# VainF/Diff-Pruning

Hardware: AMD Instinct MI355X
Metric: importance-scored images/sec (UNet fwd+bwd+|w*dL/dw|) (higher is better)
Workload: dtype f32

## Files before the change

diff-pruning_amd/_lib.py:

```python
import ctypes as C
import os

_HERE = os.path.dirname(os.path.abspath(__file__))
LIB_PATH = os.environ.get('DP_HIP_LIB') or os.path.join(_HERE, 'libdp_hip.so')

c_float_p = C.c_void_p
LL = C.c_longlong


class ConvGeom(C.Structure):
    _fields_ = [(n, C.c_int) for n in ('Ho', 'Wo', 'Hs', 'Ws', 'Hv', 'Wv', 'kw', 'stride', 'sden', 'pad_t', 'pad_l',
                                       'ups', 'c_split', '_pad')] + [('x1_img_stride', LL), ('x2_img_stride', LL)]


class ConvGemmParams(C.Structure):
    _fields_ = [('A', C.c_void_p), ('a_bs', LL), ('lda', C.c_int), ('a_kc', C.c_int),
                ('X1', C.c_void_p), ('X2', C.c_void_p), ('x_bs', LL),
                ('a_bytes', C.c_uint), ('x1_bytes', C.c_uint), ('x2_bytes', C.c_uint), ('_pad0', C.c_uint),
                ('g', ConvGeom),
                ('M', C.c_int), ('C', C.c_int), ('NPIX', C.c_int), ('ntaps', C.c_int), ('batches', C.c_int),
                ('tile', C.c_int),
                ('out', C.c_void_p), ('o_img_stride', LL), ('o_bs', LL),
                ('alpha', C.c_float), ('post_scale', C.c_float),
                ('bias', C.c_void_p), ('tadd', C.c_void_p), ('tadd_stride', LL),
                ('res', C.c_void_p), ('r_img_stride', LL),
                ('accumulate', C.c_int), ('ksplit', C.c_int), ('ws', C.c_void_p), ('x_guard', C.c_int), ('act', C.c_int),
                ('tile_counters', C.c_void_p)]


class NtGemmParams(C.Structure):
    _fields_ = [('A', C.c_void_p), ('a_bs', LL), ('a_img_stride', LL),
                ('X1', C.c_void_p), ('X2', C.c_void_p), ('x_bs', LL),
                ('a_bytes', C.c_uint), ('x1_bytes', C.c_uint), ('x2_bytes', C.c_uint), ('_pad0', C.c_uint),
                ('g', ConvGeom),
                ('M', C.c_int), ('C', C.c_int), ('NCOLS', C.c_int), ('ntaps', C.c_int), ('P', C.c_int),
                ('batches', C.c_int), ('splits', C.c_int), ('p_per_split', C.c_int), ('tile', C.c_int),
                ('batched', C.c_int),
                ('out', C.c_void_p), ('o_bs', LL), ('ldo', C.c_int), ('accumulate', C.c_int),
                ('alpha', C.c_float), ('merge', C.c_int), ('ocs', LL),
                ('o_tap_stride', LL), ('o_col_stride', C.c_int), ('xcd', C.c_int), ('col_bias', C.c_void_p)]


class AttentionParams(C.Structure):
    _fields_ = [('q', C.c_void_p), ('k', C.c_void_p), ('v', C.c_void_p), ('o', C.c_void_p),
                ('q_bs', LL), ('k_bs', LL), ('v_bs', LL), ('o_bs', LL),
                ('N', C.c_int), ('heads', C.c_int), ('d', C.c_int), ('dv', C.c_int), ('T', C.c_int), ('scale', C.c_float),
                ('variant', C.c_int), ('_pad', C.c_int)]


class Dropout(C.Structure):
    _fields_ = [('thr24', C.c_uint), ('scale', C.c_float), ('seed', C.c_ulonglong), ('site', C.c_uint), ('step', C.c_uint),
                ('n_off', LL), ('step_dev', C.c_void_p)]


class ScoreMember(C.Structure):
    _fields_ = [('w', C.c_void_p), ('g', C.c_void_p), ('R', C.c_int), ('C', C.c_int), ('T', C.c_int), ('dim', C.c_int),
                ('mode', C.c_int), ('blk0', C.c_int), ('full_off', LL), ('col_off', LL), ('idx_off', LL)]


class SliceItem(C.Structure):
    _fields_ = [('src', C.c_void_p), ('dst', C.c_void_p), ('R', C.c_int), ('C', C.c_int), ('T', C.c_int), ('dim', C.c_int),
                ('n_keep', C.c_int), ('blk0', C.c_int), ('nblk', C.c_int), ('_pad', C.c_int), ('keep_off', LL)]


class PackItem(C.Structure):
    _fields_ = [('W', C.c_void_p), ('dst', C.c_void_p), ('Co', C.c_int), ('Ci', C.c_int), ('taps', C.c_int), ('mode', C.c_int),
                ('ld', C.c_int), ('blk0', C.c_int), ('nblk', C.c_int), ('_pad', C.c_int)]


class Ups9Params(C.Structure):
    _fields_ = [('U', C.c_void_p), ('dy', C.c_void_p), ('dx', C.c_void_p), ('dy_img_stride', LL), ('dx_img_stride', LL),
                ('u_bytes', C.c_uint), ('dy_bytes', C.c_uint)] + [(n, C.c_int) for n in ('ldu', 'N', 'M', 'K', 'H', 'W',
                                                                                         'accumulate', 'tile')]


class ColsumItem(C.Structure):
    _fields_ = [('src', C.c_void_p), ('dst', C.c_void_p), ('N', C.c_int), ('C', C.c_int), ('wstride', C.c_int),
                ('woff', C.c_int), ('accumulate', C.c_int), ('ld', C.c_int)]


_vp, _i, _f, _ll = C.c_void_p, C.c_int, C.c_float, LL
_dr = C.POINTER(Dropout)

SIGNATURES = {
    'dp_conv_gemm': [C.POINTER(ConvGemmParams), _vp],
    'dp_conv_wino': [C.POINTER(ConvGemmParams), _vp],
    'dp_conv_wino_supported': [C.POINTER(ConvGemmParams)],
    'dp_conv_splitk_epilogue': [C.POINTER(ConvGemmParams), _vp],
    'dp_pack_weight_wino': [_vp, _i, _i, _i, _vp, _i, _vp],
    'dp_conv_wino2d': [C.POINTER(ConvGemmParams), _vp],
    'dp_conv_wino2d_supported': [C.POINTER(ConvGemmParams)],
    'dp_pack_weight_wino2d': [_vp, _i, _i, _i, _vp, _i, _vp],
    'dp_conv_wino43': [C.POINTER(ConvGemmParams), _vp],
    'dp_conv_wino43_supported': [C.POINTER(ConvGemmParams)],
    'dp_pack_weight_wino43': [_vp, _i, _i, _vp, _i, _vp],
    'dp_wgrad_wino': [C.POINTER(NtGemmParams), _vp],
    'dp_wgrad_wino2d': [C.POINTER(NtGemmParams), _vp],
    'dp_wgrad_wino2d_supported': [C.POINTER(NtGemmParams)],
    'dp_wgrad_wino_supported': [C.POINTER(NtGemmParams)],
    'dp_nt_gemm': [C.POINTER(NtGemmParams), _vp],
    'dp_splitk_reduce': [_vp, _ll, _i, _vp, _ll, _i, _vp],
    'dp_splitk_reduce_taps': [_vp, _ll, _i, _vp, _ll, _i, _i, _vp],
    'dp_pack_weight': [_vp, _i, _i, _i, _i, _vp, _i, _vp],
    'dp_pack_weight_batch': [C.POINTER(PackItem), _i, _vp],
    'dp_groupnorm_silu_fwd': [_vp, _vp, _i, _ll, _ll, _vp, _vp, _i, _i, _i, _i, _f, _i, _vp, _ll, _vp, _dr, _vp],
    'dp_groupnorm_silu_bwd': [_vp, _vp, _i, _ll, _ll, _vp, _vp, _vp, _vp, _ll, _i, _i, _i, _i, _i, _vp, _ll, _vp, _ll,
                              _vp, _ll, _vp, _dr, _vp, _vp],
    'dp_groupnorm_silu_fwd_split': [_vp, _vp, _i, _ll, _ll, _vp, _vp, _i, _i, _i, _i, _f, _i, _vp, _ll, _vp, _i, _vp, _dr,
                                    _vp],
    'dp_groupnorm_silu_bwd_split': [_vp, _vp, _i, _ll, _ll, _vp, _vp, _vp, _vp, _ll, _i, _i, _i, _i, _i, _vp, _ll, _vp, _ll,
                                    _vp, _ll, _vp, _i, _vp, _dr, _vp],
    'dp_colsum_accum': [_vp, _i, _i, _i, _i, _vp, _i, _vp],
    'dp_colsum_accum_batch': [C.POINTER(ColsumItem), _i, _vp],
    'dp_rowsum_nc': [_vp, _ll, _i, _i, _i, _vp, _vp],
    'dp_silu_fwd': [_vp, _vp, _ll, _vp],
    'dp_silu_bwd': [_vp, _vp, _vp, _ll, _i, _vp],
    'dp_axpby': [_vp, _f, _vp, _f, _ll, _vp],
    'dp_copy_strided': [_vp, _ll, _vp, _ll, _i, _ll, _i, _vp],
    'dp_attention_fwd': [C.POINTER(AttentionParams), _vp],
    'dp_attention_fwd_supported': [_i, _i, _i],
    'dp_softmax_fwd': [_vp, _vp, _ll, _i, _vp],
    'dp_softmax_bwd': [_vp, _vp, _vp, _ll, _i, _f, _vp],
    'dp_timestep_embedding': [_vp, _i, _i, _i, _f, _f, _vp, _vp],
    'dp_add_noise': [_vp, _vp, _vp, _vp, _i, _ll, _vp, _vp],
    'dp_mse_fwd_bwd': [_vp, _vp, _ll, _f, _vp, _vp, _i, _vp, _vp],
    'dp_kd_fwd_bwd': [_vp, _vp, _vp, _ll, _f, _f, _f, _vp, _vp, _i, _vp],
    'dp_kd_terms': [_vp, _i, _f, _f, _f, _vp, _vp],
    'dp_early_exit_update': [_vp, _f, _vp, _vp, _i, _vp],
    'dp_zero_if_stopped': [_vp, _ll, _vp, _vp],
    'dp_early_exit_update_ratio': [_vp, _f, _vp, _vp, _i, _vp],
    'dp_randn_philox': [_vp, _ll, _ll, C.c_ulonglong, C.c_uint, C.c_uint, _vp],
    'dp_sum_partials': [_vp, _i, _f, _vp, _vp],
    'dp_downsum2x2': [_vp, _ll, _i, _i, _i, _i, _vp, _ll, _vp],
    'dp_upsample2x': [_vp, _ll, _i, _i, _i, _i, _vp, _ll, _vp],
    'dp_interleave2x2': [_vp, _ll, _ll, _i, _i, _i, _i, _vp, _ll, _vp, _ll, _vp],
    'dp_deinterleave2x2': [_vp, _ll, _i, _i, _i, _i, _vp, _ll, _ll, _vp],
    'dp_ups_weff': [_vp, _ll, _vp, _vp],
    'dp_ups_wfold': [_vp, _ll, _vp, _i, _vp],
    'dp_ups9_u': [_vp, _ll, _vp, _vp],
    'dp_ups9_dgrad': [C.POINTER(Ups9Params), _vp],
    'dp_ups9_dgrad_supported': [C.POINTER(Ups9Params)],
    'dp_wg_reduce': [_vp, _vp, _i, _i, _i, _i, _i, _vp, _i, _vp, _vp],
    'dp_gather_add': [_vp, _vp, _i, _vp, _vp],
    'dp_group_score': [C.POINTER(ScoreMember), _i, _i, _vp, _vp, _vp, _vp],
    'dp_slice_batch': [C.POINTER(SliceItem), _i, _vp, _vp],
    'dp_sumsq_partials': [_vp, _ll, _vp, _i, _vp],
    'dp_clip_coef': [_vp, _i, _f, _vp, _vp, _vp],
    'dp_adam_ema': [_vp, _vp, _vp, _vp, _vp, _ll, _vp, _f, _f, _f, _f, _f, _f, _f, _vp],
    'dp_set_step_scalars': [_vp, _f, _f, _f, C.c_uint, _vp],
    'dp_adamw_ema': [_vp, _vp, _vp, _vp, _vp, _ll, _vp, _f, _f, _f, _f, _f, _f, _f, _f, _vp],
    'dp_embedding_bwd': [_vp, _vp, _i, _i, _vp, _vp],
    'dp_ema_update': [_vp, _vp, _ll, _f, _vp],
    'dp_adam_ema_dev': [_vp, _vp, _vp, _vp, _vp, _ll, _vp, _vp, _f, _f, _f, _f, _vp],
    'dp_ddim_step': [_vp, _vp, _vp, _f, _f, _f, _i, _f, _vp, _ll, _vp],
    'dp_ddpm_step': [_vp, _vp, _vp, _f, _f, _f, _f, _f, _i, _f, _vp, _ll, _vp],
    'dp_denoise_step': [_vp, _vp, _vp, _i, _f, _f, _f, _f, _f, _f, _vp, _vp, _ll, _vp],
    'dp_image_to_u8': [_vp, _ll, _i, _i, _i, _i, _i, _vp, _vp],
    'dp_cfg_denoise_step': [_vp, _vp, _vp, _f, _i, _vp, _vp, _vp, _f, _f, _f, _f, _f, _f, _vp, _vp, _vp, _vp, _ll, _vp],
    'dp_dropout_apply': [_vp, _ll, _vp, _ll, _i, _ll, _dr, _vp],
    'dp_dropout_mask': [_vp, _ll, _ll, _dr, _vp],
    'dp_layernorm_fwd': [_vp, _ll, _vp, _vp, _i, _i, _i, _f, _vp, _ll, _vp, _vp],
    'dp_layernorm_bwd': [_vp, _ll, _vp, _vp, _vp, _ll, _i, _i, _i, _vp, _ll, _vp, _ll, _vp, _vp],
    'dp_geglu_fwd': [_vp, _i, _ll, _vp, _vp],
    'dp_geglu_bwd': [_vp, _vp, _i, _ll, _vp, _vp],
    'dp_add_rowvec': [_vp, _ll, _vp, _i, _i, _i, _vp, _ll, _vp],
    'dp_q_sample': [_vp, _vp, _vp, _vp, _vp, _i, _ll, _vp, _vp],
    'dp_cfg_combine': [_vp, _vp, _f, _vp, _ll, _vp],
    'dp_u8_to_float': [_vp, _i, _i, _i, _i, _i, _vp, _ll, _i, C.c_uint, _i, _dr, _vp],
    'dp_pool2d': [_vp, _ll, _i, _i, _i, _i, _i, _i, _i, _i, _vp, _ll, _vp],
    'dp_resize_bilinear': [_vp, _ll, _i, _i, _i, _i, _i, _i, _f, _f, _vp, _vp],
    'dp_ssim': [_vp, _vp, _i, _i, _i, _i, _f, _vp, _vp, _vp],
    'dp_ssim_workspace': [_i, _i, _i, _i],
    'dp_mse_per_image': [_vp, _vp, _i, _ll, _vp, _vp],
    'dp_vq_blocks': [_ll],
    'dp_vq_quantize': [_vp, _ll, _i, _i, _ll, _vp, _i, _vp, _ll, _vp, _vp, _vp],
    'dp_vq_loss': [_vp, _i, C.c_double, _vp, _vp],
    'dp_replay_build': [_vp, C.POINTER(C.c_void_p)],
    'dp_replay_launch': [_vp, _vp, _vp],
    'dp_replay_info': [_vp, C.POINTER(C.c_int)],
    'dp_replay_free': [_vp],
    'dp_version': [],
    'dp_launch_count': [],
    'dp_recent_launches': [C.POINTER(C.c_char_p), _i],
}

_lib = None


class DpHipError(RuntimeError):
    code = None


def load():
    global _lib
# ... 20 lines not shown
```

diff-pruning_amd/csrc/ups9.hip:

```cpp
#include "dp_common.h"

#define U9_RSRC_FLAGS 0x00020000
#define U9_OOB 0x80000000u

__device__ __forceinline__ __amdgpu_buffer_rsrc_t u9_rsrc(const float* base, unsigned bytes) {
    return __builtin_amdgcn_make_buffer_rsrc((void*)base, 0, (int)bytes, U9_RSRC_FLAGS);
}
__device__ __forceinline__ float u9_bload(__amdgpu_buffer_rsrc_t r, unsigned byte_off) {
    asm volatile("" : "+v"(byte_off));
    return __builtin_bit_cast(float, __builtin_amdgcn_raw_buffer_load_b32(r, (int)byte_off, 0, 0));
}
__device__ __forceinline__ f32x4 u9_bload4(__amdgpu_buffer_rsrc_t r, unsigned byte_off) {
    asm volatile("" : "+v"(byte_off));
    return __builtin_bit_cast(f32x4, __builtin_amdgcn_raw_buffer_load_b128(r, (int)byte_off, 0, 0));
}

template <int BM, int BN, int KC, int WM, int WN, int OCC>
__global__ __launch_bounds__(256, OCC) void ups9_dgrad_kernel(const dp_ups9_params p) {
    constexpr int TM = BM / (32 * WM), TN = BN / (32 * WN);
    constexpr int KT = 9 * KC;
    constexpr int PT = BN * KC / 256;
    constexpr int KSTEP = 256 / BN;
    constexpr int MCH = BM / 4;
    constexpr int ACH = KT * MCH;
    constexpr int NA = (ACH + 255) / 256;
    static_assert(WM * WN == 4 && TM >= 1 && TN >= 1 && PT >= 1 && (BN * KC) % 256 == 0 && KT % 2 == 0 && BN <= 256, "tile");
    __shared__ __attribute__((aligned(16))) float As[KT * BM];
    __shared__ __attribute__((aligned(16))) float Ts[KT * BN];

    const int tid = threadIdx.x;
    const int lane = tid & 63;
    const int wave = __builtin_amdgcn_readfirstlane(tid >> 6);
    const int li = lane & 31, lk = lane >> 5;
    const int wm0 = (wave / WN) * (TM * 32), wn0 = (wave % WN) * (TN * 32);
    const int H = p.H, W = p.W, HW = H * W, W2 = 2 * W, HW4 = 4 * HW;
    const int K = p.K, M = p.M;
    const int NPIX = p.N * HW;
    const int MT = (M + BM - 1) / BM;
    const int PTILES = (NPIX + BN - 1) / BN;
    int mt, ptile;
    {
        const int b = blockIdx.x;
        if (!(PTILES & 7)) {
            const int xcd = b & 7, slot = b >> 3;
            mt = slot % MT;
            ptile = (slot / MT) * 8 + xcd;
        } else {
            mt = b % MT;
            ptile = b / MT;
        }
    }
    const int m0 = mt * BM, px0 = ptile * BN;

// ... 101 lines not shown
    }

#pragma unroll
    for (int tn = 0; tn < TN; ++tn) {
        const int pixel = px0 + wn0 + tn * 32 + li;
        if (pixel >= NPIX) continue;
        const int n = pixel / HW, rem = pixel - n * HW;
        float* o = p.dx + (long long)n * p.dx_img_stride + rem;
#pragma unroll
        for (int tm = 0; tm < TM; ++tm)
#pragma unroll
            for (int r = 0; r < 16; ++r) {
                const int row = m0 + wm0 + tm * 32 + (r & 3) + 8 * (r >> 2) + 4 * lk;
                if (row < M) {
                    float* q = o + (long long)row * HW;
                    *q = p.accumulate ? *q + acc[tm][tn][r] : acc[tm][tn][r];
                }
            }
    }
}

static const int u9_bn[3] = {32, 64, 128};

extern "C" int dp_ups9_dgrad_supported(const dp_ups9_params* pp) {
    const dp_ups9_params& p = *pp;
    if (!p.U || !p.dy || !p.dx || ((uintptr_t)p.U & 15)) return 0;
    if (p.N < 1 || p.M < 1 || p.K < 1 || p.H < 1 || p.W < 1 || p.tile < 0 || p.tile > 2) return 0;
    if (p.ldu < p.M || (p.ldu & 3)) return 0;
    const long long HW = (long long)p.H * p.W;
    const long long npix = HW * p.N;
    if (npix >= (1ll << 29)) return 0;
    if (9ll * p.K * p.ldu * 4 != (long long)p.u_bytes || p.u_bytes >= 0x80000000u) return 0;
    if (p.dy_img_stride < 4 * HW * p.K || p.dx_img_stride < HW * p.M) return 0;
    const long long dy_need = ((p.N - 1) * p.dy_img_stride + 4 * HW * p.K) * 4;
    if ((long long)p.dy_bytes < dy_need || p.dy_bytes >= 0x80000000u) return 0;
    const long long blocks = ((npix + u9_bn[p.tile] - 1) / u9_bn[p.tile]) * ((p.M + 127) / 128);
    if (blocks >= (1ll << 31)) return 0;
    return 1;
}

extern "C" int dp_ups9_dgrad(const dp_ups9_params* pp, void* stream) {
    if (!dp_ups9_dgrad_supported(pp)) return (int)hipErrorInvalidValue;
    const dp_ups9_params& p = *pp;
    const long long npix = (long long)p.N * p.H * p.W;
    const int bn = u9_bn[p.tile];
    const dim3 grid((unsigned)(((npix + bn - 1) / bn) * ((p.M + 127) / 128)));
    hipStream_t st = (hipStream_t)stream;
    if (p.tile == 0)      DP_LAUNCH((ups9_dgrad_kernel<128, 32, 8, 4, 1, 2>), grid, dim3(256), 0, st, p);
    else if (p.tile == 1) DP_LAUNCH((ups9_dgrad_kernel<128, 64, 4, 2, 2, 3>), grid, dim3(256), 0, st, p);
    else                  DP_LAUNCH((ups9_dgrad_kernel<128, 128, 4, 2, 2, 2>), grid, dim3(256), 0, st, p);
    return DP_LAUNCH_CHECK();
}

__global__ __launch_bounds__(256) void ups9_u_kernel(const float* __restrict__ w, long long M, float* __restrict__ u) {
    for (long long m = (long long)blockIdx.x * 256 + threadIdx.x; m < M; m += (long long)gridDim.x * 256) {
        float g[3][3], t[3][3];
#pragma unroll
        for (int i = 0; i < 9; ++i) g[i / 3][i % 3] = w[m * 9 + i];
#pragma unroll
        for (int c = 0; c < 3; ++c) {
            t[0][c] = g[0][c];
            t[1][c] = (g[0][c] + g[1][c]) + g[2][c];
            t[2][c] = g[2][c];
        }
#pragma unroll
        for (int a = 0; a < 3; ++a) {
            u[m * 9 + 3 * a + 0] = t[a][0];
            u[m * 9 + 3 * a + 1] = (t[a][0] + t[a][1]) + t[a][2];
            u[m * 9 + 3 * a + 2] = t[a][2];
        }
    }
}

extern "C" int dp_ups9_u(const float* w, long long M, float* u, void* stream) {
    if (M <= 0) return 0;
    long long nb = (M + 255) / 256;
    if (nb > 4096) nb = 4096;
    DP_LAUNCH(ups9_u_kernel, dim3((unsigned)nb), dim3(256), 0, (hipStream_t)stream, w, M, u);
    return DP_LAUNCH_CHECK();
}
```

diff-pruning_amd/engine.py:

```python
import os

import torch

from . import ops

_SPEC3 = ops.ConvSpec(3, 1, 1, 0)
_SPEC1 = ops.ConvSpec(1, 1, 0, 0)
_SPEC_UP = ops.ConvSpec(3, 1, 1, 1)
UPS_COPY = not os.environ.get('DP_NO_UPS_COPY')
UPS_SUBPIXEL = not os.environ.get('DP_NO_UPS_SUBPIXEL')
_UPS_SPECS = ops.UPS_CLASS_SPECS
S2_PARITY = not os.environ.get('DP_NO_S2_PARITY')
FUSE_QKV_WGRAD = not os.environ.get('DP_NO_FUSED_QKV_WGRAD')
OVERLAP_MIN_WORK = 4_000_000

RES_DIFFUSERS = dict(norm1='.norm1', conv1='.conv1', temb='.time_emb_proj', norm2='.norm2', conv2='.conv2',
                     shortcut='.conv_shortcut', dropout='.dropout')
RES_LDM = dict(norm1='.in_layers.0', conv1='.in_layers.2', temb='.emb_layers.1', norm2='.out_layers.0',
               conv2='.out_layers.3', shortcut='.skip_connection')


SIDE_KEEP_MAX_BYTES = int(float(os.environ.get('DP_SIDE_KEEP_GB', '4')) * (1 << 30))


# ... 362 lines not shown
    def replay_side_stream(self, device):
        if getattr(self, '_replay_side', None) is None or self._replay_side.device != torch.device(device):
            self._replay_side = shared_stream(device, 'replay', self.stream_slot)
        return self._replay_side

    def _join_side(self):
        if self._side is not None:
            torch.cuda.current_stream().wait_stream(self._side)
        self._side_keep.clear()
        self._side_keep_bytes = 0

    def _conv_bwd(self, name, dy, x, x2, spec, in_hw, *, need_dx=True, rows=None, dx_out=None, dx_accumulate=False,
                  alpha=1.0, dx_add=None):
        w = self.P[name + '.weight']

        if rows is None and (name + '.bias') in self.P and self._rows_src is not None and self._rows_src[0].data_ptr() == dy.data_ptr():
            rows = self._rows_of(dy)

        def param_grads(rows):
            ops.conv_wgrad(dy, x, x2, self.G[name + '.weight'], spec, alpha=alpha, accumulate=True)
            if (name + '.bias') in self.P:
                if rows is None:
                    rows = ops.rowsum_nc(dy)
                if alpha != 1.0:
                    rows = rows.contiguous()
                    rows = ops.axpby(rows, alpha, torch.empty_like(rows), 0.0)
                self._colsum(rows, rows.shape[0], rows.shape[1], 1, 0, self.G[name + '.bias'])

        side = self._side_stream(dy, x, x2, rows)
        if side is None:
            param_grads(rows)
        else:
            with torch.cuda.stream(side):
                param_grads(rows)
        if not need_dx:
            return None
        if (S2_PARITY and spec.stride == 2 and spec.k == 3 and not spec.ups and spec.pad in (0, 1) and alpha == 1.0
                and dx_out is None and in_hw[0] == 2 * dy.shape[2] and in_hw[1] == 2 * dy.shape[3]):
            packs = [self.packs.get(name, w, ('s2', ph, pw, spec.pad)) for ph in (0, 1) for pw in (0, 1)]
            return ops.conv_dgrad_s2(dy, packs, w.shape[1], spec, in_hw, add=dx_add)
        wd, ldd = self.packs.get(name, w, 1)
        wino = None
        if w.dim() == 4 and w.shape[2] == 3 and hasattr(ops, 'wino_wanted') and tuple(in_hw) == tuple(dy.shape[2:]):
            wino = self._wino_operand(name, w, 1, w.shape[1], (w.shape[0],), dy.shape[0], dy.shape[2], dy.shape[3], spec)
        dx = ops.conv_dgrad(dy, wd, ldd, w.shape[1], spec, in_hw, alpha=alpha, out=dx_out, accumulate=dx_accumulate,
                            **({'wino': wino} if wino is not None else {}))
        if dx_add is not None:
            ops.copy_strided(dx_add, dx, accumulate=True)
        return dx

    def _ups_conv_fwd(self, name, x):
        w = self.P[name + '.weight']
        N, _, H, W = x.shape
        q = ops.empty_act((4, N, w.shape[0], H, W), x.device)
        for c, spec in enumerate(_UPS_SPECS):
            wp, ld = self.packs.get(name, w, ('up', c, 0))
            ops.conv_forward(x, None, wp, ld, w.shape[0], spec, bias=self.P.get(name + '.bias'), out=q[c])
        return ops.interleave2x2(q)

    def _ups_conv_bwd(self, name, dy, x):
        w = self.P[name + '.weight']
        use9 = hasattr(ops, 'ups9_dgrad_wanted') and ops.ups9_dgrad_wanted(x.shape[0], w.shape[1], w.shape[0], x.shape[2], x.shape[3])
        dyq = None if use9 else ops.deinterleave2x2(dy)
        rows = None
        if (name + '.bias') in self.P and self._rows_src is not None and self._rows_src[0].data_ptr() == dy.data_ptr():
            rows = self._rows_of(dy)

        def param_grads(rows, dyq=dyq):
            if dyq is None:
                dyq = ops.deinterleave2x2(dy)
            gweff = torch.empty((4,) + tuple(w.shape[:2]) + (2, 2), dtype=torch.float32, device=dy.device)
            for c, spec in enumerate(_UPS_SPECS):
                ops.conv_wgrad(dyq[c], x, None, gweff[c], spec, accumulate=False)
            ops.ups_wfold(gweff, self.G[name + '.weight'], accumulate=True)
            if (name + '.bias') in self.P:
                if rows is None:
                    rows = ops.rowsum_nc(dy)
                self._colsum(rows, rows.shape[0], rows.shape[1], 1, 0, self.G[name + '.bias'])

        side = self._side_stream(dy, dyq, x, rows)
        if side is None:
            param_grads(rows)
        else:
            with torch.cuda.stream(side):
                param_grads(rows)
        if use9:
            up, ldu = self.packs.get(name, w, ('up9', 0, 1))
            return ops.ups9_dgrad(dy, up, ldu, w.shape[1])
        dx = None
        for c, spec in enumerate(_UPS_SPECS):
            wd, ldd = self.packs.get(name, w, ('up', c, 1))
            dx = ops.conv_dgrad(dyq[c], wd, ldd, w.shape[1], spec, tuple(x.shape[2:]), out=dx, accumulate=c > 0)
        return dx

    def _gn_param_grads(self, name, pws):
        N, C = pws.shape[0], pws.shape[1]
        self._colsum(pws, N, C, 2, 1, self.G[name + '.weight'])
        self._colsum(pws, N, C, 2, 0, self.G[name + '.bias'])

    def resnet_fwd(self, pre, xa, xb, semb, out_scale, save, names=RES_DIFFUSERS, G=None, eps=None):
        P, cfg = self.P, self.cfg
        G = cfg['norm_num_groups'] if G is None else G
        eps = cfg['norm_eps'] if eps is None else eps
        nm = names
        n1, st1 = ops.groupnorm_fwd(xa, xb, P[pre + nm['norm1'] + '.weight'], P[pre + nm['norm1'] + '.bias'], G, eps, True)
        if self._temb is not None:
# ... 334 lines not shown
```

diff-pruning_amd/ops.py:

```python
import ctypes as C
import os
import math
import torch

from . import _lib as L

_f32 = torch.float32


def _lib():
    return L.load()


_raw_stream = getattr(torch._C, '_cuda_getCurrentRawStream', None)


def _stream():
    if _raw_stream is not None:
        return C.c_void_p(_raw_stream(torch.cuda.current_device()))
    return C.c_void_p(torch.cuda.current_stream().cuda_stream)


def _p(t):
    return None if t is None else C.c_void_p(t.data_ptr())
# ... 619 lines not shown
    npix = HW * N
    if npix >= (1 << 29):
        return False
    if 9 * Cout * ldu * 4 != u_bytes or u_bytes >= _MAX_BYTES:
        return False
    if dy_img_stride < 4 * HW * Cout or dx_img_stride < HW * Cin:
        return False
    if dy_bytes < ((N - 1) * dy_img_stride + 4 * HW * Cout) * 4 or dy_bytes >= _MAX_BYTES:
        return False
    return -(-npix // UPS9_TILE_PIX[tile]) * ((Cin + 127) // 128) < (1 << 31)


def ups9_dgrad_gate(N, Cin, Cout, H, W):
    blocks32 = -(-(N * H * W) // 32) * ((Cin + 127) // 128)
    return blocks32 >= UPS9_GATE_MIN_BLOCKS and max(Cin, Cout) <= UPS9_GATE_MAX_CH


def ups9_dgrad_wanted(N, Cin, Cout, H, W):
    if not UPS9 or min(N, Cin, Cout, H, W) < 1 or N * H * W * 4 * Cout * 4 >= _MAX_BYTES:
        return False
    return ups9_dgrad_gate(N, Cin, Cout, H, W)


def _ups9_params(dy, up, ldu, Cin, out, accumulate, tile):
    sd, so = _chk_act(dy), _chk_act(out)
    N, Cout, H2, W2 = dy.shape
    p = L.Ups9Params()
    p.U, p.dy, p.dx = _p(up), _p(dy), _p(out)
    p.dy_img_stride, p.dx_img_stride = sd, so
    p.u_bytes, p.dy_bytes = up.numel() * 4, _extent_bytes(dy)
    p.ldu, p.N, p.M, p.K, p.H, p.W = ldu, N, Cin, Cout, H2 // 2, W2 // 2
    p.accumulate, p.tile = 1 if accumulate else 0, tile
    return p


def ups9_dgrad(dy, up, ldu, Cin, *, out=None, accumulate=False, tile=None):
    N, Cout, H2, W2 = dy.shape
    assert H2 % 2 == 0 and W2 % 2 == 0
    H, W = H2 // 2, W2 // 2
    if out is None:
        assert not accumulate
        out = empty_act((N, Cin, H, W), dy.device)
    assert out.shape == (N, Cin, H, W)
    if tile is None:
        tile = ups9_tile(N, Cin, H, W)
    p = _ups9_params(dy, up, ldu, Cin, out, accumulate, tile)
    ok = ups9_dgrad_shape_ok(N, Cin, Cout, H, W, p.dy_img_stride, p.dx_img_stride, p.dy_bytes, ldu, p.u_bytes, tile, up.data_ptr())
    assert ok == bool(_lib().dp_ups9_dgrad_supported(C.byref(p))), 'host shape rule and dp_ups9_dgrad_supported disagree'
    if not ok:
        raise ValueError('dp_ups9_dgrad does not take this launch (ups9_dgrad_shape_ok)')
    L.check(_run(lambda: _lib().dp_ups9_dgrad(C.byref(p), _stream()),
                 _UPS9_NAMES[tile],
                 2.0 * Cin * N * H * W * Cout * 9, 4.0 * (dy.numel() + up.numel() + out.numel())), 'dp_ups9_dgrad')
    return out


_ws_cache = {}
WGRAD_BLOCKS = 1024
WGRAD_MIN_PIX = int(os.environ.get('DP_WGRAD_MIN_PIX', '128'))


def _workspace(n, device):
    if torch.cuda.is_current_stream_capturing():
        return torch.empty(max(n, 1), dtype=_f32, device=device)
    key = (device.index if device.index is not None else torch.cuda.current_device(), _stream().value)
    t = _ws_cache.get(key)
    if t is None or t.numel() < n:
        t = torch.empty(max(n, 1 << 22), dtype=_f32, device=device)
        _ws_cache[key] = t
    return t


WGRAD_WINO = os.environ.get('DP_WGRAD_WINO', '1') not in ('0', '')
WGRAD_WINO_MIN_FILL = float(os.environ.get('DP_WGRAD_WINO_MIN_FILL', '0.7'))
WGRAD_WINO_MIN_WORK = int(os.environ.get('DP_WGRAD_WINO_MIN_WORK', '512'))


WGRAD_WINO2D = os.environ.get('DP_WGRAD_WINO2D', '1') not in ('0', '')
WGRAD_WINO2D_BLOCKS = int(os.environ.get('DP_WGRAD_WINO2D_BLOCKS', '512'))
WGRAD_WINO2D_MIN_FILL = float(os.environ.get('DP_WGRAD_WINO2D_MIN_FILL', '0.7'))


def _nt_gemm_params(A, a_img_stride, x, x2, geom, M, Cc, ncols, ntaps, P, splits, pps, tile, alpha, ldo, batch=None):
    p = L.NtGemmParams()
    Z, a_bs, x_bs, batched = batch or (1, 0, 0, 0)
    p.A, p.a_bs, p.a_img_stride = _p(A), a_bs, a_img_stride
    p.X1, p.X2, p.x_bs = _p(x), _p(x2), x_bs
    if batch is None:
        p.a_bytes, p.x1_bytes, p.x2_bytes = _extent_bytes(A), _extent_bytes(x), _extent_bytes(x2)
    else:
        p.a_bytes, p.x1_bytes, p.x2_bytes = M * P * 4, ncols * P * 4, 0
    p.g = geom
    p.M, p.C, p.NCOLS, p.ntaps, p.P = M, Cc, ncols, ntaps, P
    p.batches, p.splits, p.p_per_split, p.tile, p.batched = Z, splits, pps, tile, batched
    p.alpha, p.ldo = alpha, ldo
    return p


def _wgrad_launch(p, gw, accumulate, sym, name, flops, label, taps, device):
    acc = 1 if accumulate else 0
    if p.splits == 1:
        p.out, p.o_bs, p.accumulate = _p(gw), 0, acc
        L.check(_run(lambda: getattr(_lib(), sym)(C.byref(p), _stream()), name, flops), label)
        return gw
    n = gw.numel()
    ws = _workspace(p.splits * n, device)
# ... 894 lines not shown
```

include/dp_hip.h:

```cpp
#ifndef DP_HIP_H
#define DP_HIP_H
#include <stdint.h>
#ifdef __cplusplus
extern "C" {
#endif

typedef struct dp_conv_geom {
    int Ho, Wo, Hs, Ws, Hv, Wv, kw, stride, sden, pad_t, pad_l, ups, c_split, _pad;
    long long x1_img_stride, x2_img_stride;
} dp_conv_geom;

typedef struct dp_conv_gemm_params {
    const float* A; long long a_bs; int lda; int a_kc;
    const float* X1; const float* X2; long long x_bs;
    unsigned a_bytes, x1_bytes, x2_bytes, _pad0;
    dp_conv_geom g;
    int M, C, NPIX, ntaps, batches, tile;
    float* out; long long o_img_stride; long long o_bs;
    float alpha; float post_scale;
    const float* bias; const float* tadd; long long tadd_stride;
    const float* res; long long r_img_stride;
    int accumulate; int ksplit;
    float* ws;
    int x_guard; int act;
// ... 87 lines not shown

int dp_axpby(const float* x, float a, float* y, float b, long long n, void* stream);
int dp_copy_strided(const float* src, long long s_stride, float* dst, long long d_stride, int N, long long per_img, int accumulate, void* stream);

int dp_softmax_fwd(const float* s, float* p, long long rows, int cols, void* stream);
typedef struct dp_attention_params {
    const float* q; const float* k; const float* v; float* o;
    long long q_bs, k_bs, v_bs, o_bs;
    int N, heads, d, dv, T;
    float scale;
    int variant;
    int _pad;
} dp_attention_params;
int dp_attention_fwd(const dp_attention_params* p, void* stream);
int dp_attention_fwd_supported(int T, int d, int dv);
int dp_softmax_bwd(const float* p, const float* dp, float* ds, long long rows, int cols, float scale, void* stream);

int dp_timestep_embedding(const float* t, int B, int dim, int flip_sin_to_cos, float freq_shift, float max_period, float* out, void* stream);

int dp_add_noise(const float* x0, const float* noise, const float* acp, const int64_t* t, int B, long long per_img, float* out, void* stream);

int dp_mse_fwd_bwd(const float* out, const float* noise, long long n, float gscale, float* dout, float* partial, int nblocks,
                   const float* stop_state, void* stream);
int dp_kd_fwd_bwd(const float* out, const float* teacher, const float* noise, long long n, float w_kd, float w_eps, float gscale,
                  float* dout, float* partial, int nblocks, void* stream);
int dp_kd_terms(const float* partial, int nblocks, float w_kd, float w_eps, float scale, float* terms, void* stream);
int dp_early_exit_update(const float* loss, float thr, float* state, float* losses, int max_steps, void* stream);
int dp_zero_if_stopped(float* x, long long n, const float* state, void* stream);
int dp_early_exit_update_ratio(const float* loss, float thr, float* state, float* losses, int max_steps, void* stream);
int dp_sum_partials(const float* partial, int n, float scale, float* dst, void* stream);

int dp_downsum2x2(const float* dy, long long dy_img_stride, int N, int C, int H, int W, float* dx, long long dx_img_stride, void* stream);

int dp_upsample2x(const float* x, long long x_img_stride, int N, int C, int H, int W, float* y, long long y_img_stride, void* stream);

int dp_interleave2x2(const float* q, long long q_class_stride, long long q_img_stride, int N, int C, int Ho, int Wo,
                     const float* add, long long add_img_stride, float* dx, long long dx_img_stride, void* stream);

int dp_deinterleave2x2(const float* y, long long y_img_stride, int N, int C, int Ho, int Wo, float* q,
                       long long q_class_stride, long long q_img_stride, void* stream);

int dp_ups_weff(const float* w, long long M, float* weff, void* stream);
int dp_ups_wfold(const float* gweff, long long M, float* gw, int accumulate, void* stream);

typedef struct dp_ups9_params {
    const float* U; const float* dy; float* dx;
    long long dy_img_stride, dx_img_stride;
    unsigned u_bytes, dy_bytes;
    int ldu, N, M, K, H, W, accumulate, tile;
} dp_ups9_params;
int dp_ups9_u(const float* w, long long M, float* u, void* stream);
int dp_ups9_dgrad(const dp_ups9_params* p, void* stream);
int dp_ups9_dgrad_supported(const dp_ups9_params* p);

int dp_wg_reduce(const float* w, const float* g, int R, int C, int T, int dim, int mode, float* out, int accumulate,
                 float* scratch, void* stream);

int dp_gather_add(const float* src, const int64_t* idx, int n, float* dst, void* stream);

typedef struct dp_score_member {
    const float* w; const float* g;
    int R, C, T, dim, mode, blk0;
    long long full_off, col_off, idx_off;
} dp_score_member;
int dp_group_score(const dp_score_member* members, int n, int n0, const int64_t* idx, float* scratch, float* score, void* stream);
typedef struct dp_slice_item {
    const float* src; float* dst;
    int R, C, T, dim, n_keep, blk0, nblk, _pad;
    long long keep_off;
} dp_slice_item;
int dp_slice_batch(const dp_slice_item* items, int n, const int64_t* keep, void* stream);

int dp_sumsq_partials(const float* x, long long n, float* partial, int nblocks, void* stream);
int dp_set_step_scalars(float* hyper, float lr, float bc1, float bc2, unsigned step, void* stream);
int dp_adam_ema_dev(float* p, const float* g, float* m, float* v, float* ema, long long n, const float* clip_coef,
                    const float* hyper, float b1, float b2, float eps, float ema_decay, void* stream);
int dp_clip_coef(const float* partial, int n, float max_norm, float* norm_out, float* coef_out, void* stream);
int dp_adam_ema(float* p, const float* g, float* m, float* v, float* ema, long long n, const float* clip_coef,
                float lr, float b1, float b2, float eps, float bc1, float bc2, float ema_decay, void* stream);

int dp_adamw_ema(float* p, const float* g, float* m, float* v, float* ema, long long n, const float* clip_coef,
                 float p_scale, float one_minus_b1, float b2, float one_minus_b2, float sqrt_bc2, float eps,
                 float step_size, float ema_decay, void* stream);
int dp_ema_update(float* s, const float* p, long long n, float one_minus_decay, void* stream);
int dp_embedding_bwd(const long long* ids, const float* dctx, int B, int D, float* dW, void* stream);

int dp_ddim_step(const float* x, const float* eps, const float* vnoise, float a_t, float a_prev, float std, int clip,
                 float clip_range, float* out, long long n, void* stream);

int dp_ddpm_step(const float* x, const float* eps, const float* vnoise, float sqrt_a_t, float sqrt_b_t, float c_x0,
                 float c_xt, float sigma, int clip, float clip_range, float* out, long long n, void* stream);

#define DP_DENOISE_MAX_BLOCKS 4096
int dp_denoise_step(const float* x, const float* eps, const float* z, int mode, float p0, float p1, float p2, float p3, float p4,
                    float p5, float* next, float* x0_out, long long n, void* stream);
int dp_image_to_u8(const float* x, long long x_img_stride, int N, int C, int H, int W, int rescaled, unsigned char* out,
                   void* stream);

int dp_cfg_denoise_step(const float* x, const float* e_u, const float* e_c, float scale, int order, const float* h1, const float* h2,
                        const float* h3, float s1m, float sqrt_a_t, float sqrt_a_prev, float c_dir, float sigma, float temperature,
                        const float* z, float* next, float* x0_out, float* eg_out, long long n, void* stream);

int dp_layernorm_fwd(const float* x, long long x_img_stride, const float* gamma, const float* beta, int N, int C, int T,
                     float eps, float* y, long long y_img_stride, float* stats, void* stream);
int dp_layernorm_bwd(const float* x, long long x_img_stride, const float* gamma, const float* stats, const float* dy,
                     long long dy_img_stride, int N, int C, int T, float* dx, long long dx_img_stride, const float* add,
// ... 46 lines not shown
```

Before: 4953.

## Add Winograd-style fused upsample+conv3x3 forward kernel for small-channel layers

Adds a HIP kernel that computes nearest-2x-upsample followed by a 3x3 conv in one pass. It transforms a 3x3 input neighbourhood into 9 Winograd-like terms, multiplies them by pre-transformed weights with MFMA, and writes the 2x2 output pixels directly. This replaces the previous path that ran four per-class GEMMs into an intermediate q buffer and then interleaved them. The new path is gated by block count and channel limits. It adds a pack type ('up9') and extra LDS pressure, and any layer that fails the gate falls back to the old path.

Result: faster. 5017 (median of 6 runs) (+1.3%).

```diff
diff --git a/diff-pruning_amd/_lib.py b/diff-pruning_amd/_lib.py
--- a/diff-pruning_amd/_lib.py
+++ b/diff-pruning_amd/_lib.py
@@ -72,6 +72,11 @@
     _fields_ = [('U', C.c_void_p), ('dy', C.c_void_p), ('dx', C.c_void_p), ('dy_img_stride', LL), ('dx_img_stride', LL),
                 ('u_bytes', C.c_uint), ('dy_bytes', C.c_uint)] + [(n, C.c_int) for n in ('ldu', 'N', 'M', 'K', 'H', 'W',
                                                                                          'accumulate', 'tile')]
+
+
+class Ups9FwdParams(C.Structure):
+    _fields_ = [('U', C.c_void_p), ('x', C.c_void_p), ('bias', C.c_void_p), ('y', C.c_void_p), ('x_img_stride', LL), ('y_img_stride', LL),
+                ('u_bytes', C.c_uint), ('x_bytes', C.c_uint)] + [(n, C.c_int) for n in ('ldu', 'N', 'M', 'K', 'H', 'W')]
 
 
 class ColsumItem(C.Structure):
@@ -140,6 +145,7 @@
     'dp_ups9_u': [_vp, _ll, _vp, _vp],
     'dp_ups9_dgrad': [C.POINTER(Ups9Params), _vp],
     'dp_ups9_dgrad_supported': [C.POINTER(Ups9Params)],
+    'dp_ups9_fwd': [C.POINTER(Ups9FwdParams), _vp],
     'dp_wg_reduce': [_vp, _vp, _i, _i, _i, _i, _i, _vp, _i, _vp, _vp],
     'dp_gather_add': [_vp, _vp, _i, _vp, _vp],
     'dp_group_score': [C.POINTER(ScoreMember), _i, _i, _vp, _vp, _vp, _vp],
diff --git a/diff-pruning_amd/csrc/ups9.hip b/diff-pruning_amd/csrc/ups9.hip
--- a/diff-pruning_amd/csrc/ups9.hip
+++ b/diff-pruning_amd/csrc/ups9.hip
@@ -1,4 +1,6 @@
 #include "dp_common.h"
+
+typedef float f32x2 __attribute__((ext_vector_type(2)));
 
 #define U9_RSRC_FLAGS 0x00020000
 #define U9_OOB 0x80000000u
@@ -206,6 +208,190 @@
     return DP_LAUNCH_CHECK();
 }
 
+template <int BM, int BN, int KC, int OCC>
+__global__ __launch_bounds__(256, OCC) void ups9_fwd_kernel(const dp_ups9_fwd_params p) {
+    constexpr int WN = BN / 32;
+    constexpr int KT = 9 * KC;
+    constexpr int PT = BN * KC / 256;
+    constexpr int KSTEP = 256 / BN;
+    constexpr int MCH = BM / 4;
+    constexpr int ACH = KT * MCH;
+    constexpr int NA = (ACH + 255) / 256;
+    constexpr int NS = 9 * KC / 2;
+    static_assert((BM / 32) * WN == 4 && PT >= 1 && BN * KC % 256 == 0 && KC % 2 == 0 && BM % 32 == 0 && BN % 32 == 0, "tile");
+    __shared__ __attribute__((aligned(16))) float As[KT * BM];
+    __shared__ __attribute__((aligned(16))) float Vs[KT * BN];
+
+    const int tid = threadIdx.x;
+    const int lane = tid & 63;
+    const int wave = __builtin_amdgcn_readfirstlane(tid >> 6);
+    const int li = lane & 31, lk = lane >> 5;
+    const int wm0 = (wave / WN) * 32, wn0 = (wave % WN) * 32;
+    const int H = p.H, W = p.W, HW = H * W;
+    const int K = p.K, M = p.M;
+    const int NPIX = p.N * HW;
+    const int MT = (M + BM - 1) / BM;
+    const int PTILES = (NPIX + BN - 1) / BN;
+    int mt, ptile;
+    {
+        const int b = blockIdx.x;
+        if (!(PTILES & 7)) {
+            const int xcd = b & 7, slot = b >> 3;
+            mt = slot % MT;
+            ptile = (slot / MT) * 8 + xcd;
+        } else {
+            mt = b % MT;
+            ptile = b / MT;
+        }
+    }
+    const int m0 = mt * BM, px0 = ptile * BN;
+
+    const int ppix = tid % BN, pk0 = tid / BN;
+    int pbase;
+    bool pvalid, top, bot, left, right;
+    {
+        const int pixel = px0 + ppix;
+        pvalid = pixel < NPIX;
+        const int n = pixel / HW, rem = pixel - n * HW;
+        const int i = rem / W, j = rem - i * W;
+        pbase = (int)(n * p.x_img_stride) + (i - 1) * W + (j - 1);
+        top = i > 0, bot = i < H - 1, left = j > 0, right = j < W - 1;
+    }
+    const __amdgpu_buffer_rsrc_t rA = u9_rsrc(p.U, p.u_bytes);
+    const __amdgpu_buffer_rsrc_t rB = u9_rsrc(p.x, p.x_bytes);
+
+    float pr[PT][9];
+    f32x4 ar[NA];
+    auto load_tile = [&](int k0) {
+#pragma unroll
+        for (int j = 0; j < NA; ++j) {
+            const int e = tid + 256 * j;
+            const int kk = e / MCH, m = m0 + 4 * (e % MCH);
+            const int tap = kk / KC, k = k0 + kk % KC;
+            const bool v = e < ACH && m < p.ldu && k < K;
+            ar[j] = u9_bload4(rA, v ? (unsigned)(((tap * K + k) * p.ldu + m) * 4) : U9_OOB);
+        }
+#pragma unroll
+        for (int q = 0; q < PT; ++q) {
+            const int k = k0 + pk0 + KSTEP * q;
+            const bool ok = pvalid && k < K;
+            const int off0 = pbase + k * HW;
+#pragma unroll
+            for (int r = 0; r < 3; ++r) {
+                const bool rok = ok && (r == 0 ? top : r == 2 ? bot : true);
+#pragma unroll
+                for (int c = 0; c < 3; ++c) {
+                    const bool v = rok && (c == 0 ? left : c == 2 ? right : true);
+                    pr[q][3 * r + c] = u9_bload(rB, v ? (unsigned)((off0 + r * W + c) * 4) : U9_OOB);
+                }
+            }
+        }
+    };
+    auto store_tile = [&]() {
+#pragma unroll
+        for (int j = 0; j < NA; ++j)
+            if (NA * 256 == ACH || tid + 256 * j < ACH) *(f32x4*)&As[(tid + 256 * j) * 4] = ar[j];
+#pragma unroll
+        for (int q = 0; q < PT; ++q) {
+            const float* d = pr[q];
+            float t[3][3];
+#pragma unroll
+            for (int c = 0; c < 3; ++c) {
+                t[0][c] = d[c] - d[3 + c];
+                t[1][c] = d[3 + c];
+                t[2][c] = d[6 + c] - d[3 + c];
+            }
+            const int kc = pk0 + KSTEP * q;
+#pragma unroll
+            for (int a = 0; a < 3; ++a) {
+                Vs[((3 * a + 0) * KC + kc) * BN + ppix] = t[a][0] - t[a][1];
+                Vs[((3 * a + 1) * KC + kc) * BN + ppix] = t[a][1];
+                Vs[((3 * a + 2) * KC + kc) * BN + ppix] = t[a][2] - t[a][1];
+            }
+        }
+    };
+
+    f32x16 acc[9];
+#pragma unroll
+    for (int t = 0; t < 9; ++t)
+#pragma unroll
+        for (int r = 0; r < 16; ++r) acc[t][r] = 0.f;
+
+    const int nIter = (K + KC - 1) / KC;
+    load_tile(0);
+    for (int it = 0; it < nIter; ++it) {
+        __syncthreads();
+        store_tile();
+        __syncthreads();
+        if (it + 1 < nIter) load_tile((it + 1) * KC);
+        float a[3], b[3];
+        auto frag = [&](int s, float& fa, float& fb) {
+            const int kk = (s % 9) * KC + (s / 9) * 2 + lk;
+            fa = As[kk * BM + wm0 + li];
+            fb = Vs[kk * BN + wn0 + li];
+        };
+        frag(0, a[0], b[0]);
+        frag(1, a[1], b[1]);
+#pragma unroll
+        for (int s = 0; s < NS; ++s) {
+            if (s + 2 < NS) frag(s + 2, a[(s + 2) % 3], b[(s + 2) % 3]);
+            __builtin_amdgcn_sched_barrier(0);
+            acc[s % 9] = __builtin_amdgcn_mfma_f32_32x32x2f32(a[s % 3], b[s % 3], acc[s % 9], 0, 0, 0);
+            __builtin_amdgcn_sched_barrier(0);
+        }
+    }
+
+    const int pixel = px0 + wn0 + li;
+    if (pixel >= NPIX) return;
+    const int n = pixel / HW, rem = pixel - n * HW;
+    const int i = rem / W, j = rem - i * W;
+    float* o = p.y + (long long)n * p.y_img_stride + (long long)(2 * i) * (2 * W) + 2 * j;
+#pragma unroll
+    for (int r = 0; r < 16; ++r) {
+        const int row = m0 + wm0 + (r & 3) + 8 * (r >> 2) + 4 * lk;
+        if (row < M) {
+            const float bv = p.bias ? p.bias[row] : 0.f;
+            const float c0 = acc[0][r] + acc[3][r], c1 = acc[1][r] + acc[4][r], c2 = acc[2][r] + acc[5][r];
+            const float d0 = acc[3][r] + acc[6][r], d1 = acc[4][r] + acc[7][r], d2 = acc[5][r] + acc[8][r];
+            float* q = o + (long long)row * (4 * HW);
+            f32x2 y0, y1;
+            y0[0] = (c0 + c1) + bv, y0[1] = (c1 + c2) + bv;
+            y1[0] = (d0 + d1) + bv, y1[1] = (d1 + d2) + bv;
+            *(f32x2*)q = y0;
+            *(f32x2*)(q + 2 * W) = y1;
+        }
+    }
+}
+
+#define U9F_BM 64
+#define U9F_BN 64
+
+static bool u9f_ok(const dp_ups9_fwd_params& p) {
+    if (!p.U || !p.x || !p.y || ((uintptr_t)p.U & 15) || ((uintptr_t)p.y & 7) || ((uintptr_t)p.bias & 3)) return false;
+    if (p.N < 1 || p.M < 1 || p.K < 1 || p.H < 1 || p.W < 1) return false;
+    if (p.ldu < p.M || (p.ldu & 3)) return false;
+    const long long HW = (long long)p.H * p.W;
+    const long long npix = HW * p.N;
+    if (npix >= (1ll << 29)) return false;
+    if (9ll * p.K * p.ldu * 4 != (long long)p.u_bytes || p.u_bytes >= 0x80000000u) return false;
+    if (p.x_img_stride < HW * p.K || p.y_img_stride < 4 * HW * p.M || (p.y_img_stride & 1)) return false;
+    const long long x_need = ((p.N - 1) * p.x_img_stride + HW * p.K) * 4;
+    if ((long long)p.x_bytes < x_need || p.x_bytes >= 0x80000000u) return false;
+    const long long blocks = ((npix + U9F_BN - 1) / U9F_BN) * ((p.M + U9F_BM - 1) / U9F_BM);
+    if (blocks >= (1ll << 31)) return false;
+    return true;
+}
+
+extern "C" int dp_ups9_fwd(const dp_ups9_fwd_params* pp, void* stream) {
+    const dp_ups9_fwd_params& p = *pp;
+    if (!u9f_ok(p)) return (int)hipErrorInvalidValue;
+    const long long npix = (long long)p.N * p.H * p.W;
+    const dim3 grid((unsigned)(((npix + U9F_BN - 1) / U9F_BN) * ((p.M + U9F_BM - 1) / U9F_BM)));
+    static_assert(U9F_BM == 64 && U9F_BN == 64, "the launch below names its tile");
+    DP_LAUNCH((ups9_fwd_kernel<64, 64, 8, 2>), grid, dim3(256), 0, (hipStream_t)stream, p);
+    return DP_LAUNCH_CHECK();
+}
+
 __global__ __launch_bounds__(256) void ups9_u_kernel(const float* __restrict__ w, long long M, float* __restrict__ u) {
     for (long long m = (long long)blockIdx.x * 256 + threadIdx.x; m < M; m += (long long)gridDim.x * 256) {
         float g[3][3], t[3][3];
diff --git a/diff-pruning_amd/engine.py b/diff-pruning_amd/engine.py
--- a/diff-pruning_amd/engine.py
+++ b/diff-pruning_amd/engine.py
@@ -438,6 +438,9 @@
     def _ups_conv_fwd(self, name, x):
         w = self.P[name + '.weight']
         N, _, H, W = x.shape
+        if hasattr(ops, 'ups9_fwd_wanted') and ops.ups9_fwd_wanted(N, w.shape[1], w.shape[0], H, W):
+            up, ldu = self.packs.get(name, w, ('up9', 0, 0))
+            return ops.ups9_fwd(x, up, ldu, w.shape[0], bias=self.P.get(name + '.bias'))
         q = ops.empty_act((4, N, w.shape[0], H, W), x.device)
         for c, spec in enumerate(_UPS_SPECS):
             wp, ld = self.packs.get(name, w, ('up', c, 0))
diff --git a/diff-pruning_amd/ops.py b/diff-pruning_amd/ops.py
--- a/diff-pruning_amd/ops.py
+++ b/diff-pruning_amd/ops.py
@@ -695,6 +695,71 @@
     L.check(_run(lambda: _lib().dp_ups9_dgrad(C.byref(p), _stream()),
                  _UPS9_NAMES[tile],
                  2.0 * Cin * N * H * W * Cout * 9, 4.0 * (dy.numel() + up.numel() + out.numel())), 'dp_ups9_dgrad')
+    return out
+
+
+UPS9_FWD_TILE = (64, 64)
+_UPS9_FWD_NAME = 'ups9_fwd_kernel<64, 64, 8, 2>'
+UPS9_FWD_GATE_MIN_BLOCKS, UPS9_FWD_GATE_MAX_CH = 96, 256
+
+
+def ups9_fwd_shape_ok(N, Cin, Cout, H, W, x_img_stride, y_img_stride, x_bytes, ldu, u_bytes, u_ptr=0, y_ptr=0, bias_ptr=0):
+    if min(N, Cin, Cout, H, W) < 1 or (u_ptr & 15) or (y_ptr & 7) or (bias_ptr & 3):
+        return False
+    if ldu < Cout or (ldu & 3):
+        return False
+    HW = H * W
+    npix = HW * N
+    if npix >= (1 << 29):
+        return False
+    if 9 * Cin * ldu * 4 != u_bytes or u_bytes >= _MAX_BYTES:
+        return False
+    if x_img_stride < HW * Cin or y_img_stride < 4 * HW * Cout or (y_img_stride & 1):
+        return False
+    if x_bytes < ((N - 1) * x_img_stride + HW * Cin) * 4 or x_bytes >= _MAX_BYTES:
+        return False
+    bm, bn = UPS9_FWD_TILE
+    return -(-npix // bn) * -(-Cout // bm) < (1 << 31)
+
+
+def ups9_fwd_gate(N, Cin, Cout, H, W):
+    bm, bn = UPS9_FWD_TILE
+    blocks = -(-(N * H * W) // bn) * -(-Cout // bm)
+    return blocks >= UPS9_FWD_GATE_MIN_BLOCKS and max(Cin, Cout) <= UPS9_FWD_GATE_MAX_CH
+
+
+def ups9_fwd_wanted(N, Cin, Cout, H, W):
+    if not UPS9 or min(N, Cin, Cout, H, W) < 1 or N * H * W * max(Cin, 4 * Cout) * 4 >= _MAX_BYTES:
+        return False
+    return ups9_fwd_gate(N, Cin, Cout, H, W)
+
+
+def _ups9_fwd_params(x, up, ldu, Cout, bias, out):
+    sx, so = _chk_act(x), _chk_act(out)
+    N, Cin, H, W = x.shape
+    p = L.Ups9FwdParams()
+    p.U, p.x, p.bias, p.y = _p(up), _p(x), _p(bias), _p(out)
+    p.x_img_stride, p.y_img_stride = sx, so
+    p.u_bytes, p.x_bytes = up.numel() * 4, _extent_bytes(x)
+    p.ldu, p.N, p.M, p.K, p.H, p.W = ldu, N, Cout, Cin, H, W
+    return p
+
+
+def ups9_fwd(x, up, ldu, Cout, *, bias=None, out=None):
+    N, Cin, H, W = x.shape
+    if out is None:
+        out = empty_act((N, Cout, 2 * H, 2 * W), x.device)
+    assert out.shape == (N, Cout, 2 * H, 2 * W) and (bias is None or (bias.numel() == Cout and bias.is_contiguous()))
+    p = _ups9_fwd_params(x, up, ldu, Cout, bias, out)
+    ok = ups9_fwd_shape_ok(N, Cin, Cout, H, W, p.x_img_stride, p.y_img_stride, p.x_bytes, ldu, p.u_bytes, up.data_ptr(),
+                           out.data_ptr(), bias.data_ptr() if bias is not None else 0)
+    if not ok:
+        raise ValueError('dp_ups9_fwd does not take this launch (ups9_fwd_shape_ok)')
+    rc = _run(lambda: _lib().dp_ups9_fwd(C.byref(p), _stream()),
+              _UPS9_FWD_NAME,
+              2.0 * Cin * N * H * W * Cout * 9, 4.0 * (x.numel() + up.numel() + out.numel()))
+    assert rc != 1, 'host shape rule and dp_ups9_fwd disagree (hipErrorInvalidValue for a launch ups9_fwd_shape_ok takes)'
+    L.check(rc, 'dp_ups9_fwd')
     return out
 
 
diff --git a/include/dp_hip.h b/include/dp_hip.h
--- a/include/dp_hip.h
+++ b/include/dp_hip.h
@@ -163,6 +163,13 @@
 int dp_ups9_u(const float* w, long long M, float* u, void* stream);
 int dp_ups9_dgrad(const dp_ups9_params* p, void* stream);
 int dp_ups9_dgrad_supported(const dp_ups9_params* p);
+typedef struct dp_ups9_fwd_params {
+    const float* U; const float* x; const float* bias; float* y;
+    long long x_img_stride, y_img_stride;
+    unsigned u_bytes, x_bytes;
+    int ldu, N, M, K, H, W;
+} dp_ups9_fwd_params;
+int dp_ups9_fwd(const dp_ups9_fwd_params* p, void* stream);
 
 int dp_wg_reduce(const float* w, const float* g, int R, int C, int T, int dim, int mode, float* out, int accumulate,
                  float* scratch, void* stream);
```
